# isarandi/metrabs

Hardware: AMD Instinct MI355X
Metric: crops/sec (256px, 72 depth bins) at 1/2/4/8 MI355X; MPJPE vs ref (higher is better)
Workload: dtype f32

## Files before the change

include/metrabs_hip.h:

```cpp
#ifndef METRABS_HIP_H_
#define METRABS_HIP_H_

#include <stddef.h>
#include <stdint.h>

#ifdef __cplusplus
extern "C" {
#endif

#define MTR_VERSION 100

typedef void* mtr_stream_t;

enum mtr_dtype { MTR_F32 = 0, MTR_F16 = 1, MTR_BF16 = 2 };

enum mtr_layout {
  MTR_NCHW = 0,
  MTR_NHWC = 1
};

enum mtr_error {
  MTR_OK = 0,
  MTR_E_NULL = -1,
  MTR_E_SHAPE = -2,
// ... 62 lines not shown
  MTR_HEAD_KERNEL_RT_KS = 3,
  MTR_HEAD_KERNEL_RT_NP = 4,
  MTR_HEAD_KERNEL_16 = 10,
  MTR_HEAD_KERNEL_16_DMA = 11,
  MTR_HEAD_KERNEL_16_DMA_EARLY = 14,
  MTR_HEAD_KERNEL_16_DMA_LOADER = 13,
  MTR_HEAD_KERNEL_16_AREG = 15,
  MTR_HEAD_KERNEL_16_RES = 16,
  MTR_HEAD_KERNEL_16_PP = 17,
  MTR_HEAD_KERNEL_16_DMA_EARLY_TIGHT = 18,
  MTR_HEAD_KERNEL_16_RT = 12
};
typedef struct mtr_head_plan_info {
  int32_t kernel;
  int32_t tiles_per_workgroup;
  int32_t column_blocks;
  int32_t split_column_blocks;
  int64_t workgroups;
  double model_us;
} mtr_head_plan_info;
int mtr_head_plan(int feat_dtype, int layout, int B, int C, int H, int W, int J, int D,
                  const mtr_head_options* options, int have_workspace, mtr_head_plan_info* plan);

size_t mtr_head_workspace_bytes(int feat_dtype, int layout, int B, int C, int H, int W, int J, int D);
int mtr_head_fused_ws(const void* features, int feat_dtype, int layout, int B, int C, int H, int W,
                      const void* packed, int J, int D, const mtr_head_params* p,
                      const mtr_head_options* options, void* workspace, size_t workspace_bytes,
                      float* coords2d, float* coords3d_rel, mtr_stream_t stream);

size_t mtr_reconstruct_workspace_bytes(int B, int J);
int mtr_reconstruct_absolute(const float* coords2d , const float* coords3d_rel ,
                             const float* intrinsics , int B, int J,
                             const mtr_recon_params* p, float* poses3d , void* workspace,
                             size_t workspace_bytes, mtr_stream_t stream);
int mtr_reconstruct_moments(const float* coords2d, const float* coords3d_rel,
                            const float* intrinsics, int B, int J, double* moments ,
                            void* workspace, size_t workspace_bytes, mtr_stream_t stream);
int mtr_reconstruct_solve(const float* coords2d, const float* coords3d_rel, const float* intrinsics,
                          int B, int J, const mtr_recon_params* p, const double* moments ,
                          float* poses3d, mtr_stream_t stream);

#define MTR_WARP_PARAM_FLOATS 36

int mtr_build_pyramid(const uint8_t* images_u8, int N, int Hi, int Wi, float* level0, float* level1,
                      float* level2, mtr_stream_t stream);
int mtr_pyramid_from_level0(const float* level0, int N, int Hi, int Wi, float* level1, float* level2,
                            mtr_stream_t stream);
int mtr_build_pyramid_u8(const uint8_t* images_u8, int N, int Hi, int Wi, float* lut ,
                         float* level1, float* level2, mtr_stream_t stream);
int mtr_warp_crops_u8(const uint8_t* level0_u8, const float* lut, const float* level1,
                      const float* level2, int N, int Hi, int Wi, const float* warp_params,
                      int n_crops, int res, int antialias, int out_dtype, int out_layout, void* out,
                      mtr_stream_t stream);
int mtr_build_pyramid_u8_hwc(const uint8_t* images_u8, int N, int Hi, int Wi, float* lut ,
                             float* level1, float* level2, mtr_stream_t stream);
int mtr_warp_crops_u8_hwc(const uint8_t* level0_u8, const float* lut, const float* level1,
                          const float* level2, int N, int Hi, int Wi, const float* warp_params,
                          int n_crops, int res, int antialias, int out_dtype, int out_layout, void* out,
                          mtr_stream_t stream);
int mtr_crop_geometry(const float* boxes, int box_stride, const float* intrinsics,
                      const float* distortion, const float* camspace_up, const int32_t* image_ids,
                      const float* aug_rotflipmat, const float* aug_scales, const float* aug_gammas,
                      int n_box, int n_aug, int res, int antialias, float* new_intrinsics,
                      float* rot, float* warp_params, mtr_stream_t stream);
int mtr_warp_crops(const float* level0, const float* level1, const float* level2, int N, int Hi,
                   int Wi, const float* warp_params, int n_crops, int res, int antialias,
                   int out_dtype, int out_layout, void* out, mtr_stream_t stream);
size_t mtr_crops_shrink_workspace_bytes(int n_crops, int res, int antialias);
int mtr_crops_shrink_antialiased(const float* crops_big, const float* warp_params, int n_crops, int res,
                                 int antialias, int out_dtype, int out_layout, void* out,
                                 void* workspace, size_t workspace_bytes, mtr_stream_t stream);

int mtr_postprocess_poses(const float* poses_crop, const float* rot, const uint8_t* should_flip,
                          const int32_t* mirror_mapping, const float* joint_transform, int Jt,
                          const int32_t* skeleton, int S, const float* intrinsics,
                          const float* distortion, const float* inv_extrinsics, int A, int n, int J,
                          int average_aug, float* poses3d, float* poses2d, mtr_stream_t stream);

int mtr_linear_combine_points(const float* points, const float* weights, int B, int J_in, int J_out,
                              float* out, mtr_stream_t stream);

typedef struct mtr_detector_geom {
  int32_t target_h, target_w;
  int32_t antialias;
  int32_t pad_top, pad_left;
  int32_t out_h, out_w;
  float x_factor, y_factor;
} mtr_detector_geom;

int mtr_detector_geometry(int H, int W, int input_size , mtr_detector_geom* g);
int mtr_detector_preprocess(const uint8_t* images_u8, int N, int H, int W, const mtr_detector_geom* g,
                            float* out, mtr_stream_t stream);
enum { MTR_DETECTOR_KERNEL_AUTO = 0, MTR_DETECTOR_KERNEL_TILE = 1, MTR_DETECTOR_KERNEL_STREAM = 2 };
int mtr_detector_preprocess_kernel(const uint8_t* images_u8, int N, int H, int W, const mtr_detector_geom* g,
                                   int kernel, float* out, mtr_stream_t stream);
int mtr_detector_scale_boxes(const float* xyxy_conf, int n, const mtr_detector_geom* g,
                             float* boxes_out, mtr_stream_t stream);

typedef struct mtr_filter_params {
  float rel_small, rel_big, abs_diff_mm;
  float stdev_mm;
  float box_fraction;
  float sim_scale_mm, sim_threshold;
  int32_t max_output;
  int32_t var_correction;
  int32_t order_by_score;
} mtr_filter_params;

size_t mtr_filter_poses_workspace_bytes(int P, int J, int max_per_image);
int mtr_filter_poses(const float* poses3d, const float* poses2d, const float* boxes,
                     const int32_t* row_start, const int32_t* sim_offsets, int n_images, int P, int A,
                     int J, const int32_t* edges, const float* mean_bones, int n_bones, int J_model,
                     const mtr_filter_params* params , void* workspace, size_t workspace_bytes,
                     int max_per_image, uint8_t* valid, int32_t* keep_idx, int32_t* keep_count,
                     mtr_stream_t stream);

int mtr_bias_act_nchw(void* y, int dtype, const float* bias , const void* residual, int act,
                      long long B, int C, int HW, mtr_stream_t stream);

int mtr_bias_act_rowmean_nchw(void* y, int dtype, const float* bias , int act, long long B,
                              int C, int HW, float* row_mean , mtr_stream_t stream);

int mtr_depthwise3x3_bias_act(const void* x, int dtype, const float* weight, const float* bias, int act,
                              long long B, int C, int H, int W, int stride, int pad, void* y,
                              float* row_mean, mtr_stream_t stream);
int mtr_depthwise3x3_bias_act_padded(const void* x, int dtype, const float* weight, const float* bias,
                                     int act, long long B, int C, int H, int W, int stride, int pad_top,
                                     int pad_left, int pad_bottom, int pad_right, void* y,
                                     float* row_mean, mtr_stream_t stream);

int mtr_depthwise5x5_bias_act_padded(const void* x, int dtype, const float* weight ,
                                     const float* bias, int act, long long B, int C, int H, int W,
                                     int stride, int pad_top, int pad_left, int pad_bottom, int pad_right,
                                     void* y, float* row_mean , mtr_stream_t stream);

int mtr_se_gate(const float* mean , const float* w1, const float* b1, const float* w2,
                const float* b2, int act, int gate_fn, int B, int C, int S, float* gate ,
                mtr_stream_t stream);

int mtr_conv1x1_bias_act(const void* x, int dtype, const float* weight, const float* bias,
                         const float* gate , const void* residual, int act, long long B,
                         int M, int K, int HW, void* y, mtr_stream_t stream);

int mtr_conv1x1_bias_act16(const void* x, int dtype, const void* weight, const float* bias,
                           const float* gate , const void* residual, int act, long long B,
                           int M, int K, int HW, void* y, mtr_stream_t stream);

int mtr_conv3x3_bias_act16(const void* x, int dtype, const void* weight , const float* bias,
                           const void* residual, int act, long long B, int Cin, int Cout, int H, int W, int stride,
                           void* y, mtr_stream_t stream);

size_t mtr_conv3x3_16_lds_bytes(long long B, int Cin, int Cout, int H, int W, int stride);

#ifdef __cplusplus
}
#endif
#endif
```

metrabs_amd/_lib.py:

```python
import ctypes
import os
from ctypes import POINTER, c_char_p, c_double, c_float, c_int, c_int32, c_size_t, c_uint8, c_void_p

LIB_PATH = os.path.join(os.path.dirname(os.path.abspath(__file__)), 'csrc', 'libmetrabs_hip.so')

MTR_F32, MTR_F16, MTR_BF16 = 0, 1, 2
MTR_NCHW, MTR_NHWC = 0, 1
MTR_WARP_PARAM_FLOATS = 36


class HeadParams(ctypes.Structure):
    _fields_ = [('proc_side', c_int32), ('stride_test', c_int32), ('centered_stride', c_int32),
                ('legacy_centered_stride_bug', c_int32), ('box_size_mm', c_float)]


class HeadOptions(ctypes.Structure):
    _fields_ = [('struct_size', ctypes.c_uint32),
                ('rt_tiles_per_workgroup', c_int32), ('groups_per_workgroup', c_int32),
                ('dma_staging', c_int32), ('rt_column_blocks', c_int32), ('rt_k_groups', c_int32),
                ('rt_loader', c_int32), ('rt_split_column_blocks', c_int32)]


def head_options(rt_tiles=0, groups_per_workgroup=0, dma_staging=-1, rt_column_blocks=0, rt_k_groups=0,
                 rt_loader=0, rt_split=0):
    return HeadOptions(ctypes.sizeof(HeadOptions), int(rt_tiles), int(groups_per_workgroup), int(dma_staging),
                       int(rt_column_blocks), int(rt_k_groups), int(rt_loader), int(rt_split))


class HeadPlanInfo(ctypes.Structure):
    _fields_ = [('kernel', c_int32), ('tiles_per_workgroup', c_int32), ('column_blocks', c_int32),
                ('split_column_blocks', c_int32), ('workgroups', ctypes.c_int64), ('model_us', ctypes.c_double)]


HEAD_KERNEL_NAMES = {1: 'head_rt_kernel', 2: 'head_rt_ld_kernel', 3: 'head_rt_ks_kernel', 4: 'head_rt_np_kernel',
                     10: 'head_fused16_kernel', 11: 'head_fused16dma_kernel', 12: 'head_rt16_kernel',
                     13: 'head_fused16dma_kernel (loader wave)', 14: 'head_fused16dma_kernel (early copies)',
                     15: 'head_fused16areg_kernel (weights in registers)',
                     16: 'head_fused16res_kernel (weights resident, persistent workgroups)',
                     17: 'head_fused16pp_kernel (two alternating halves)',
                     18: 'head_fused16dma_kernel (early copies, tight stage)'}


class ReconParams(ctypes.Structure):
    _fields_ = [('proc_side', c_int32), ('stride_train', c_int32), ('centered_stride', c_int32),
                ('weak_perspective', c_int32), ('mix_enabled', c_int32),
                ('mix_3d_inside_fov', c_float), ('l2_reg', c_float), ('weight_eps', c_float),
                ('fov_border_factor', c_float)]


class DetectorGeom(ctypes.Structure):
    _fields_ = [('target_h', c_int32), ('target_w', c_int32), ('antialias', c_int32),
                ('pad_top', c_int32), ('pad_left', c_int32), ('out_h', c_int32), ('out_w', c_int32),
                ('x_factor', c_float), ('y_factor', c_float)]


class FilterParams(ctypes.Structure):
    _fields_ = [('rel_small', c_float), ('rel_big', c_float), ('abs_diff_mm', c_float),
                ('stdev_mm', c_float), ('box_fraction', c_float), ('sim_scale_mm', c_float),
                ('sim_threshold', c_float), ('max_output', c_int32), ('var_correction', c_int32),
                ('order_by_score', c_int32)]


SIGNATURES = {
    'mtr_version': (c_int, []),
    'mtr_strerror': (c_char_p, [c_int]),
    'mtr_softargmax_decode': (c_int, [c_void_p, c_int, c_int, c_int, c_int, c_int, c_int, c_int,
                                      POINTER(HeadParams), c_void_p, c_void_p, c_void_p]),
    'mtr_softargmax_decode_opts': (c_int, [c_void_p, c_int, c_int, c_int, c_int, c_int, c_int, c_int,
                                           POINTER(HeadParams), c_int, c_void_p, c_void_p, c_void_p]),
    'mtr_head_row_plan': (c_int, [c_int, c_int, POINTER(c_int32), POINTER(c_int32), c_void_p, c_int]),
    'mtr_head_packed_bytes': (c_size_t, [c_int, c_int, c_int, c_int]),
    'mtr_head_pack_weights': (c_int, [c_void_p, c_void_p, c_int, c_int, c_int, c_int, c_void_p,
                                      c_void_p]),
    'mtr_head_fused': (c_int, [c_void_p, c_int, c_int, c_int, c_int, c_int, c_int, c_void_p, c_int,
                               c_int, POINTER(HeadParams), c_void_p, c_void_p, c_void_p]),
    'mtr_head_fused_opts': (c_int, [c_void_p, c_int, c_int, c_int, c_int, c_int, c_int, c_void_p, c_int,
                                    c_int, POINTER(HeadParams), POINTER(HeadOptions), c_void_p, c_void_p,
                                    c_void_p]),
    'mtr_head_plan': (c_int, [c_int, c_int, c_int, c_int, c_int, c_int, c_int, c_int, POINTER(HeadOptions),
                              c_int, POINTER(HeadPlanInfo)]),
    'mtr_head_workspace_bytes': (c_size_t, [c_int, c_int, c_int, c_int, c_int, c_int, c_int, c_int]),
    'mtr_head_fused_ws': (c_int, [c_void_p, c_int, c_int, c_int, c_int, c_int, c_int, c_void_p, c_int,
                                  c_int, POINTER(HeadParams), POINTER(HeadOptions), c_void_p, c_size_t,
                                  c_void_p, c_void_p, c_void_p]),
    'mtr_crops_shrink_workspace_bytes': (c_size_t, [c_int, c_int, c_int]),
    'mtr_crops_shrink_antialiased': (c_int, [c_void_p, c_void_p, c_int, c_int, c_int, c_int, c_int, c_void_p,
                                             c_void_p, c_size_t, c_void_p]),
    'mtr_reconstruct_workspace_bytes': (c_size_t, [c_int, c_int]),
    'mtr_reconstruct_absolute': (c_int, [c_void_p, c_void_p, c_void_p, c_int, c_int,
                                         POINTER(ReconParams), c_void_p, c_void_p, c_size_t,
                                         c_void_p]),
    'mtr_reconstruct_moments': (c_int, [c_void_p, c_void_p, c_void_p, c_int, c_int, c_void_p,
                                        c_void_p, c_size_t, c_void_p]),
    'mtr_reconstruct_solve': (c_int, [c_void_p, c_void_p, c_void_p, c_int, c_int,
                                      POINTER(ReconParams), c_void_p, c_void_p, c_void_p]),
    'mtr_build_pyramid': (c_int, [c_void_p, c_int, c_int, c_int, c_void_p, c_void_p, c_void_p,
                                  c_void_p]),
    'mtr_build_pyramid_u8': (c_int, [c_void_p, c_int, c_int, c_int, c_void_p, c_void_p, c_void_p,
                                     c_void_p]),
    'mtr_warp_crops_u8': (c_int, [c_void_p, c_void_p, c_void_p, c_void_p, c_int, c_int, c_int, c_void_p,
                                  c_int, c_int, c_int, c_int, c_int, c_void_p, c_void_p]),
    'mtr_build_pyramid_u8_hwc': (c_int, [c_void_p, c_int, c_int, c_int, c_void_p, c_void_p, c_void_p,
                                         c_void_p]),
    'mtr_warp_crops_u8_hwc': (c_int, [c_void_p, c_void_p, c_void_p, c_void_p, c_int, c_int, c_int, c_void_p,
                                      c_int, c_int, c_int, c_int, c_int, c_void_p, c_void_p]),
    'mtr_pyramid_from_level0': (c_int, [c_void_p, c_int, c_int, c_int, c_void_p, c_void_p, c_void_p]),
    'mtr_crop_geometry': (c_int, [c_void_p, c_int, c_void_p, c_void_p, c_void_p, c_void_p, c_void_p,
                                  c_void_p, c_void_p, c_int, c_int, c_int, c_int, c_void_p,
                                  c_void_p, c_void_p, c_void_p]),
    'mtr_postprocess_poses': (c_int, [c_void_p, c_void_p, c_void_p, c_void_p, c_void_p, c_int, c_void_p,
                                      c_int, c_void_p, c_void_p, c_void_p, c_int, c_int, c_int, c_int,
                                      c_void_p, c_void_p, c_void_p]),
    'mtr_linear_combine_points': (c_int, [c_void_p, c_void_p, c_int, c_int, c_int, c_void_p, c_void_p]),
    'mtr_warp_crops': (c_int, [c_void_p, c_void_p, c_void_p, c_int, c_int, c_int, c_void_p, c_int,
                               c_int, c_int, c_int, c_int, c_void_p, c_void_p]),
    'mtr_detector_geometry': (c_int, [c_int, c_int, c_int, POINTER(DetectorGeom)]),
    'mtr_detector_preprocess': (c_int, [c_void_p, c_int, c_int, c_int, POINTER(DetectorGeom), c_void_p,
                                        c_void_p]),
    'mtr_detector_preprocess_kernel': (c_int, [c_void_p, c_int, c_int, c_int, POINTER(DetectorGeom), c_int,
                                               c_void_p, c_void_p]),
    'mtr_detector_scale_boxes': (c_int, [c_void_p, c_int, POINTER(DetectorGeom), c_void_p, c_void_p]),
    'mtr_filter_poses_workspace_bytes': (ctypes.c_size_t, [c_int, c_int, c_int]),
    'mtr_filter_poses': (c_int, [c_void_p, c_void_p, c_void_p, c_void_p, c_void_p, c_int, c_int, c_int,
                                 c_int, c_void_p, c_void_p, c_int, c_int, POINTER(FilterParams), c_void_p,
                                 ctypes.c_size_t, c_int, c_void_p, c_void_p, c_void_p, c_void_p]),
    'mtr_depthwise3x3_bias_act': (c_int, [c_void_p, c_int, c_void_p, c_void_p, c_int, ctypes.c_longlong,
                                          c_int, c_int, c_int, c_int, c_int, c_void_p, c_void_p, c_void_p]),
    'mtr_depthwise3x3_bias_act_padded': (c_int, [c_void_p, c_int, c_void_p, c_void_p, c_int, ctypes.c_longlong,
                                                 c_int, c_int, c_int, c_int, c_int, c_int, c_int, c_int,
                                                 c_void_p, c_void_p, c_void_p]),
    'mtr_depthwise5x5_bias_act_padded': (c_int, [c_void_p, c_int, c_void_p, c_void_p, c_int, ctypes.c_longlong,
                                                 c_int, c_int, c_int, c_int, c_int, c_int, c_int, c_int,
                                                 c_void_p, c_void_p, c_void_p]),
    'mtr_bias_act_rowmean_nchw': (c_int, [c_void_p, c_int, c_void_p, c_int, ctypes.c_longlong, c_int, c_int,
                                          c_void_p, c_void_p]),
    'mtr_bias_act_nchw': (c_int, [c_void_p, c_int, c_void_p, c_void_p, c_int, ctypes.c_longlong, c_int,
                                  c_int, c_void_p]),
    'mtr_se_gate': (c_int, [c_void_p, c_void_p, c_void_p, c_void_p, c_void_p, c_int, c_int, c_int, c_int,
                            c_int, c_void_p, c_void_p]),
    'mtr_conv1x1_bias_act': (c_int, [c_void_p, c_int, c_void_p, c_void_p, c_void_p, c_void_p, c_int,
                                     ctypes.c_longlong, c_int, c_int, c_int, c_void_p, c_void_p]),
    'mtr_conv1x1_bias_act16': (c_int, [c_void_p, c_int, c_void_p, c_void_p, c_void_p, c_void_p, c_int,
                                       ctypes.c_longlong, c_int, c_int, c_int, c_void_p, c_void_p]),
    'mtr_conv3x3_bias_act16': (c_int, [c_void_p, c_int, c_void_p, c_void_p, c_void_p, c_int, ctypes.c_longlong,
                                       c_int, c_int, c_int, c_int, c_int, c_void_p, c_void_p]),
    'mtr_conv3x3_16_lds_bytes': (ctypes.c_size_t, [ctypes.c_longlong, c_int, c_int, c_int, c_int, c_int]),
}

_lib = None


def load(path=None):
    global _lib
    if _lib is not None and path is None:
        return _lib
    path = path or LIB_PATH
    import torch
    if not os.path.exists(path):
        raise RuntimeError(
            f'{path} not found: the HIP extension is not built. Run `python -m metrabs_amd.build` '
            f'(needs hipcc). metrabs_amd has no CPU fallback.')
    lib = ctypes.CDLL(path)
    for name, (restype, argtypes) in SIGNATURES.items():
        fn = getattr(lib, name)
        fn.restype = restype
        fn.argtypes = argtypes
    _lib = lib
    return lib


def check(code, what):
    if code != 0:
        msg = load().mtr_strerror(code).decode()
        raise RuntimeError(f'{what} failed: {msg} (code {code})')


def dtype_code(torch_dtype):
    import torch
    try:
        return {torch.float32: MTR_F32, torch.float16: MTR_F16, torch.bfloat16: MTR_BF16}[torch_dtype]
    except KeyError:
        raise TypeError(f'unsupported dtype {torch_dtype}') from None


def current_stream_ptr(device=None):
    import torch
    return c_void_p(torch.cuda.current_stream(device).cuda_stream)


def require_cuda(*tensors):
    for t in tensors:
        if t is not None and not t.is_cuda:
            raise RuntimeError(
                'metrabs_amd kernels run on the GPU only (tensor on %s); there is no CPU fallback'
                % t.device)
```

metrabs_amd/backbones.py:

```python
import collections
import threading

import torch
import torch.nn.functional as F
from torch import nn


class DepthwiseConv2d(nn.Conv2d):

    use_miopen = False
    _backend_lock = threading.Lock()

    def forward(self, x):
        if x.is_cuda and not DepthwiseConv2d.use_miopen and torch.backends.cudnn.enabled:
            cudnn = torch.backends.cudnn
            with DepthwiseConv2d._backend_lock, cudnn.flags(
                    enabled=False, benchmark=cudnn.benchmark, deterministic=cudnn.deterministic,
                    allow_tf32=cudnn.allow_tf32):
                return super().forward(x)
        return super().forward(x)


class ConvBNAct(nn.Sequential):

# ... 207 lines not shown
        return mobilenet_v3_large()
    raise ValueError(f'unknown backbone {name}')


_ACT_NAMES = {nn.SiLU: 'silu', nn.ReLU: 'relu', nn.Hardswish: 'hardswish'}


class ConvBiasAct(nn.Module):

    def __init__(self, conv, bias, act):
        super().__init__()
        self.conv = conv
        self.register_buffer('bias', bias.detach().float().contiguous())
        self.act = act
        self.act_name = None if act is None else _ACT_NAMES[type(act)]
        self.emit_mean = False
        self._mean = None
        self._gate = None
        self.last_path = None

    use_k13 = True
    k13_slower = frozenset({(960, 256, 64), (1536, 256, 64), (256, 1280, 64)})

    def k13_takes(self, x):
        c = self.conv
        if not (ConvBiasAct.use_k13 and not self.emit_mean and x.is_cuda and c.kernel_size == (1, 1)
                and c.stride == (1, 1) and c.padding == (0, 0) and c.dilation == (1, 1) and c.groups == 1
                and c.bias is None and c.padding_mode == 'zeros'):
            return False
        if torch.is_autocast_enabled('cuda') or (torch.is_grad_enabled() and c.weight.requires_grad):
            return False
        if x.dim() != 4 or (c.in_channels, c.out_channels, x.shape[2] * x.shape[3]) in ConvBiasAct.k13_slower:
            return False
        from . import kernels
        return kernels.conv1x1_supported(x, c.weight)

    use_k13h = True
    k13h_slower = frozenset({(192, 48, 4096), (256, 64, 1024), (1536, 256, 64), (256, 64, 9216), (768, 192, 576),
                             (1152, 224, 576), (1344, 224, 576), (1344, 384, 144), (2304, 384, 144),
                             (2304, 640, 144), (640, 3840, 144), (3840, 640, 144), (640, 1280, 144)})

    def k13h_takes(self, x):
        c = self.conv
        if not (ConvBiasAct.use_k13h and not self.emit_mean and x.is_cuda and x.dtype == c.weight.dtype
                and x.dtype in (torch.float16, torch.bfloat16) and c.kernel_size == (1, 1)
                and c.stride == (1, 1) and c.padding == (0, 0) and c.dilation == (1, 1) and c.groups == 1
                and c.bias is None and c.padding_mode == 'zeros'):
            return False
        if torch.is_autocast_enabled('cuda') or (torch.is_grad_enabled() and c.weight.requires_grad):
            return False
        if x.dim() != 4 or (c.in_channels, c.out_channels, x.shape[2] * x.shape[3]) in ConvBiasAct.k13h_slower:
            return False
        from . import kernels
        return kernels.conv1x1_16_supported(x, c.weight)

    def give_gate(self, x, gate):
        self._gate = (x, gate)

    def take_mean_f32(self, x):
        held, self._mean = self._mean, None
        if held is not None and held[0] is x:
            return held[1]
        return None

    def take_mean(self, x):
        m = self.take_mean_f32(x)
        return None if m is None else m.to(x.dtype).view(x.shape[0], x.shape[1], 1, 1)

    def forward(self, x, residual=None):
        held, self._gate = self._gate, None
        gate = held[1] if held is not None and held[0] is x else None
        w16 = self.conv.weight.dtype
        if x.dtype != w16 and w16 in (torch.float16, torch.bfloat16) and not torch.is_autocast_enabled(x.device.type):
            x = x.to(w16)
        if self.k13h_takes(x) and (residual is None or (residual.dtype == x.dtype and residual.is_contiguous()
                                                        and residual.data_ptr() % 16 == 0)):
            from . import kernels
            self.last_path = 'k13h' if gate is None else 'k13h_gate'
            return kernels.conv1x1_bias_act16(x, self.conv.weight, self.bias, self.act_name, gate=gate,
                                              residual=residual)
        if self.k13_takes(x) and (residual is None or (residual.dtype == x.dtype and residual.is_contiguous()
                                                       and residual.data_ptr() % 16 == 0)):
            from . import kernels
            self.last_path = 'k13' if gate is None else 'k13_gate'
            return kernels.conv1x1_bias_act(x, self.conv.weight, self.bias, self.act_name, gate=gate,
                                            residual=residual)
        self.last_path = 'library'
        if gate is not None:
            x = x * gate.to(x.dtype).view(x.shape[0], x.shape[1], 1, 1)
        return _library_conv_bias_act(self, x, residual)


def _library_conv_bias_act(mod, x, residual):
    y = mod.conv(x)
    hw_vec_ok = (y.shape[2] * y.shape[3]) % (16 // y.element_size()) == 0
    if y.is_cuda and y.is_contiguous() and hw_vec_ok and y.data_ptr() % 16 == 0 and (
            residual is None or (residual.dtype == y.dtype and residual.is_contiguous()
                                 and residual.data_ptr() % 16 == 0)):
        from . import kernels
        if getattr(mod, 'emit_mean', False) and residual is None:
            y, mean = kernels.bias_act_rowmean_(y, mod.bias, mod.act_name)
            mod._mean = (y, mean)
            return y
        return kernels.bias_act_(y, mod.bias, mod.act_name, residual)
    y = y + mod.bias.view(1, -1, 1, 1).to(y.dtype)
    y = y if mod.act is None else mod.act(y)
    return y if residual is None else residual + y


class Conv3x3BiasAct(nn.Module):

    use_k14h = True
    k14h_slower = frozenset({(64, 256, 2, 96, 96), (64, 64, 1, 64, 64)})

    def __init__(self, conv, bias, act):
        super().__init__()
        self.conv = conv
        from . import kernels
        self.register_buffer('weight_packed', kernels.pack_conv3x3_weight(conv.weight))
        self.register_buffer('bias', bias.detach().float().contiguous())
        self.act = act
        self.act_name = None if act is None else _ACT_NAMES[type(act)]
        self.stride = conv.stride[0]
        self.last_path = None

    @staticmethod
    def applies_to(conv):
        return (isinstance(conv, nn.Conv2d) and conv.groups == 1 and conv.kernel_size == (3, 3)
                and conv.dilation == (1, 1) and conv.stride in ((1, 1), (2, 2)) and conv.padding == (1, 1)
                and conv.padding_mode == 'zeros' and conv.in_channels % 8 == 0)

    def k14h_takes(self, x):
        c = self.conv
        if not (Conv3x3BiasAct.use_k14h and x.is_cuda and x.dim() == 4 and x.dtype == c.weight.dtype
                and x.dtype in (torch.float16, torch.bfloat16) and c.bias is None):
            return False
        if torch.is_autocast_enabled('cuda') or (torch.is_grad_enabled() and c.weight.requires_grad):
            return False
        if (c.in_channels, c.out_channels, self.stride, x.shape[2], x.shape[3]) in Conv3x3BiasAct.k14h_slower:
            return False
        from . import kernels
        return kernels.conv3x3_16_supported(x, self.weight_packed, self.stride)

    def forward(self, x, residual=None):
        w16 = self.conv.weight.dtype
        if x.dtype != w16 and w16 in (torch.float16, torch.bfloat16) and not torch.is_autocast_enabled(x.device.type):
            x = x.to(w16)
        if self.k14h_takes(x) and (residual is None or (residual.dtype == x.dtype and residual.is_contiguous()
                                                        and residual.data_ptr() % 16 == 0)):
            from . import kernels
            self.last_path = 'k14h'
            return kernels.conv3x3_bias_act16(x, self.weight_packed, self.bias, self.act_name, self.stride,
                                              residual=residual)
        self.last_path = 'library'
        return _library_conv_bias_act(self, x, residual)


class DepthwiseBiasAct(nn.Module):

    kernel_sizes = (3, 5)
    k15_slower = frozenset()

    def __init__(self, conv, bias, act):
        super().__init__()
        self.weight = nn.Parameter(conv.weight.detach().float().contiguous(), requires_grad=False)
        self.register_buffer('bias', bias.detach().float().contiguous())
        self.k = conv.kernel_size[0]
        self.stride, self.pad = conv.stride[0], conv.padding[0]
        self.pads = None
        self.act = act
        self.act_name = None if act is None else _ACT_NAMES[type(act)]
        self.emit_mean = False
        self._mean = None
        self.last_path = None

    @classmethod
    def applies_to(cls, conv):
        k = conv.kernel_size[0] if isinstance(conv, nn.Conv2d) else None
        return (isinstance(conv, nn.Conv2d) and conv.groups == conv.in_channels == conv.out_channels
                and conv.groups > 1 and k in cls.kernel_sizes and conv.kernel_size == (k, k)
                and conv.dilation == (1, 1) and conv.stride in ((1, 1), (2, 2))
                and conv.padding in ((0, 0), (k // 2, k // 2)) and conv.padding_mode == 'zeros')

    take_mean = ConvBiasAct.take_mean
    take_mean_f32 = ConvBiasAct.take_mean_f32

    def forward(self, x):
        pl, pr = (self.pad, self.pad) if self.pads is None else self.pads[:2]
        ow = (x.shape[3] + pl + pr - self.k) // self.stride + 1
        pad = self.pad if self.pads is None else self.pads
        if x.is_cuda and x.is_contiguous() and ow % 4 == 0 and \
                x.dtype in (torch.float32, torch.float16, torch.bfloat16):
            from . import kernels
            if self.k == 3:
                fn, self.last_path = kernels.depthwise3x3_bias_act, 'k11'
            elif (x.shape[1], x.shape[2], x.shape[3], self.stride) not in DepthwiseBiasAct.k15_slower and \
                    kernels.depthwise5x5_supported(x.shape[2], x.shape[3], pad):
                fn, self.last_path = kernels.depthwise5x5_bias_act, 'k15'
            else:
                fn = None
            if fn is not None:
                if self.emit_mean:
                    y, mean = fn(x, self.weight, self.bias, self.act_name, self.stride, pad, want_mean=True)
                    self._mean = (y, mean)
                    return y
                return fn(x, self.weight, self.bias, self.act_name, self.stride, pad)
        self.last_path = 'library'
        if self.pads is not None:
            x = F.pad(x, self.pads)
        y = F.conv2d(x, self.weight.to(x.dtype), self.bias.to(x.dtype), self.stride,
                     self.pad if self.pads is None else 0, groups=self.weight.shape[0])
        return y if self.act is None else self.act(y)


def _block_plus_skip(block, x):
    last = block[-1]
    tail = last[0] if isinstance(last, ConvBNAct) else None
    if isinstance(tail, (ConvBiasAct, Conv3x3BiasAct)):
        y = x
        for m in list(block)[:-1]:
            y = m(y)
        for m in list(last)[1:]:
            assert isinstance(m, nn.Identity)
        return tail(y, residual=x)
    return x + block(x)


def fold_batchnorm(backbone, fused_epilogue=False, dtype=None):
    import copy
    from torch.nn.utils.fusion import fuse_conv_bn_eval
    if backbone.training:
        raise ValueError('fold_batchnorm needs the running statistics of an eval-mode network')
    if dtype not in (None, torch.float16, torch.bfloat16):
        raise ValueError(f'fold_batchnorm: dtype must be None, torch.float16 or torch.bfloat16, got {dtype}')
    if dtype is not None and not fused_epilogue:
        raise ValueError('fold_batchnorm: a 16-bit copy (dtype=) needs fused_epilogue=True')
    folded = copy.deepcopy(backbone)
    for m in folded.modules():
        if isinstance(m, ConvBNAct) and isinstance(m[1], nn.BatchNorm2d):
            conv = fuse_conv_bn_eval(m[0], m[1])
            act = m[2] if len(m) > 2 else None
            if fused_epilogue and (act is None or type(act) in _ACT_NAMES):
                bias, conv.bias = conv.bias, None
                m[0] = (DepthwiseBiasAct if DepthwiseBiasAct.applies_to(conv) else ConvBiasAct)(
                    conv, bias, act)
                if act is not None:
                    m[2] = nn.Identity()
            else:
                m[0] = conv
            m[1] = nn.Identity()
    if any(isinstance(m, nn.BatchNorm2d) for m in folded.modules()):
        raise ValueError('a BatchNorm2d outside a ConvBNAct block cannot be folded here')
    if fused_epilogue:
        for seq in folded.modules():
            if not isinstance(seq, nn.Sequential) or isinstance(seq, ConvBNAct):
                continue
            names = list(seq._modules)
            for n_pad, n_conv in zip(names, names[1:]):
                pad, blk = seq._modules[n_pad], seq._modules[n_conv]
                if isinstance(pad, nn.ZeroPad2d) and isinstance(blk, ConvBNAct) and \
                        isinstance(blk[0], DepthwiseBiasAct) and blk[0].pad == 0:
                    l, r, t, b = (int(p) for p in pad.padding)
                    lo, hi = blk[0].k // 2, blk[0].k // 2 + 1
                    if 0 <= l <= lo and 0 <= t <= lo and 0 <= r <= hi and 0 <= b <= hi:
                        blk[0].pads = (l, r, t, b)
                        seq._modules[n_pad] = nn.Identity()
    if fused_epilogue:
        for seq in folded.modules():
            if not isinstance(seq, nn.Sequential) or isinstance(seq, ConvBNAct):
                continue
            kids = list(seq)
            for prev, nxt in zip(kids, kids[1:]):
                if isinstance(nxt, SqueezeExcite) and isinstance(prev, ConvBNAct) and \
                        isinstance(prev[0], (ConvBiasAct, DepthwiseBiasAct)) and \
                        all(isinstance(m, nn.Identity) for m in list(prev)[1:]):
                    prev[0].emit_mean = True
                    nxt.mean_from = (prev[0],)
        for seq in folded.modules():
            if not isinstance(seq, nn.Sequential) or isinstance(seq, ConvBNAct):
                continue
            kids = list(seq)
            for prev, nxt in zip(kids, kids[1:]):
                if isinstance(prev, SqueezeExcite) and isinstance(nxt, ConvBNAct) and \
                        isinstance(nxt[0], ConvBiasAct):
                    prev.gate_to = (nxt[0],)
    if dtype is not None:
        for m in folded.modules():
            if isinstance(m, ConvBiasAct):
                m.conv.to(dtype)
        for m in folded.modules():
            if isinstance(m, ConvBNAct) and isinstance(m[0], ConvBiasAct) and not m[0].emit_mean \
                    and Conv3x3BiasAct.applies_to(m[0].conv):
                m[0] = Conv3x3BiasAct(m[0].conv, m[0].bias, m[0].act)
        folded.inference_dtype = dtype
    return folded


def calibrate_batchnorm(backbone, res, dev, batches=2, batch_size=16, seed=7, samples=None):
    bns = [m for m in backbone.modules() if isinstance(m, torch.nn.BatchNorm2d)]
    for m in bns:
        m.momentum = None
        m.reset_running_stats()
    backbone.train()
    g = torch.Generator(device=dev).manual_seed(seed)
    with torch.no_grad():
        for _ in range(batches):
            backbone(torch.rand(batch_size, 3, res, res, device=dev, generator=g))
        if samples is not None:
            for chunk in samples.float().split(batch_size):
                if len(chunk) > 1:
                    backbone(chunk)
    backbone.eval()
    return backbone
```

metrabs_amd/kernels.py:

```python
import ctypes

import torch

from metrabs_amd import _lib
from metrabs_amd._lib import check, current_stream_ptr, dtype_code, require_cuda


def _ptr(t):
    return ctypes.c_void_p(t.data_ptr()) if t is not None else ctypes.c_void_p(0)


def softargmax_decode(logits, n_points, cfg, out=None, nhwc_staging=0):
    require_cuda(logits)
    lib = _lib.load()
    nhwc = _is_channels_last(logits)
    if not nhwc:
        logits = logits.contiguous()
    B, n_out, H, W = logits.shape
    J = int(n_points)
    D = n_out // J - 1
    if n_out != J * (1 + D) or D != cfg.depth:
        raise ValueError(f'logits have {n_out} channels, expected J*(1+depth) = {J * (1 + cfg.depth)}')
    if out is None:
        c2d = torch.empty(B, J, 2, device=logits.device, dtype=torch.float32)
# ... 488 lines not shown


def depthwise5x5_bias_act(x, weight, bias, act, stride, pad, want_mean=False):
    require_cuda(x, weight, bias)
    if not x.is_contiguous():
        raise ValueError('depthwise5x5_bias_act needs an NCHW-contiguous tensor')
    if weight.numel() != x.shape[1] * 25:
        raise ValueError(f'depthwise5x5_bias_act needs a [C, 5, 5] weight, got {tuple(weight.shape)}')
    B, C, H, W = x.shape
    pl, pr, pt, pb = (pad,) * 4 if isinstance(pad, int) else tuple(int(p) for p in pad)
    OH, OW = (H + pt + pb - 5) // stride + 1, (W + pl + pr - 5) // stride + 1
    y = torch.empty(B, C, max(OH, 0), max(OW, 0), device=x.device, dtype=x.dtype)
    mean = torch.empty(B, C, device=x.device, dtype=torch.float32) if want_mean else None
    check(_lib.load().mtr_depthwise5x5_bias_act_padded(
        _ptr(x), dtype_code(x.dtype), _ptr(weight.contiguous().float()), _ptr(bias.contiguous().float()),
        ACT_CODES[act], B, C, H, W, int(stride), pt, pl, pb, pr, _ptr(y), None if mean is None else _ptr(mean),
        current_stream_ptr(x.device)), 'mtr_depthwise5x5_bias_act_padded')
    return (y, mean) if want_mean else y



SE_GATE_CODES = {'sigmoid': 0, 'hardsigmoid': 1}


def se_gate(mean, w1, b1, w2, b2, act, gate_fn, out=None):
    require_cuda(mean, w1, b1, w2, b2)
    B, C = mean.shape[0], mean.shape[1]
    S = w1.shape[0]
    w1, w2 = w1.reshape(S, -1), w2.reshape(C, -1)
    if mean.dtype != torch.float32 or mean.numel() != B * C or w1.shape[1] != C or w2.shape[1] != S:
        raise ValueError('se_gate: mean [B, C] f32, w1 [S, C], w2 [C, S]')
    tensors = [t.contiguous().float() for t in (mean, w1, b1, w2, b2)]
    if out is None:
        out = torch.empty(B, C, device=mean.device, dtype=torch.float32)
    check(_lib.load().mtr_se_gate(*(_ptr(t) for t in tensors), ACT_CODES[act], SE_GATE_CODES[gate_fn], B, C, S,
                                  _ptr(out), current_stream_ptr(mean.device)), 'mtr_se_gate')
    return out



def conv1x1_supported(x, weight):
    if x.dim() != 4 or x.dtype != torch.float32 or weight.dtype != torch.float32 or not x.is_contiguous():
        return False
    K, HW = x.shape[1], x.shape[2] * x.shape[3]
    return (weight.numel() == weight.shape[0] * K and HW % 4 == 0 and K % 4 == 0
            and x.data_ptr() % 16 == 0 and weight.data_ptr() % 16 == 0
            and x.shape[0] * HW < 2 ** 31 and K * HW < 2 ** 31 and weight.shape[0] * HW < 2 ** 31)


def conv1x1_bias_act(x, w, bias, act, gate=None, residual=None, out=None):
    require_cuda(x, w, bias, gate, residual)
    B, K, H, W = x.shape
    M = w.shape[0]
    w = w.reshape(M, -1)
    if w.shape[1] != K:
        raise ValueError(f'conv1x1_bias_act: weight has {w.shape[1]} input channels, x has {K}')
    if gate is not None and (gate.dtype != torch.float32 or gate.numel() != B * K):
        raise ValueError('conv1x1_bias_act: gate must be [B, Cin] f32')
    if residual is not None and (residual.shape != (B, M, H, W) or residual.dtype != x.dtype
                                 or not residual.is_contiguous()):
        raise ValueError('conv1x1_bias_act: residual must be [B, Cout, H, W] like the output, contiguous')
    if out is None:
        out = torch.empty(B, M, H, W, device=x.device, dtype=x.dtype)
    elif out.shape != (B, M, H, W) or out.dtype != x.dtype or not out.is_contiguous():
        raise ValueError('conv1x1_bias_act: out must be [B, Cout, H, W] like the output, contiguous')
    check(_lib.load().mtr_conv1x1_bias_act(
        _ptr(x), dtype_code(x.dtype), _ptr(w.contiguous()), _ptr(bias.contiguous().float()),
        None if gate is None else _ptr(gate.contiguous()), None if residual is None else _ptr(residual),
        ACT_CODES[act], B, M, K, H * W, _ptr(out), current_stream_ptr(x.device)), 'mtr_conv1x1_bias_act')
    return out



def conv1x1_16_supported(x, weight):
    if x.dim() != 4 or x.dtype not in (torch.float16, torch.bfloat16) or weight.dtype != x.dtype \
            or not x.is_contiguous() or not weight.is_contiguous():
        return False
    K, HW = x.shape[1], x.shape[2] * x.shape[3]
    return (weight.numel() == weight.shape[0] * K and HW % 8 == 0 and K % 8 == 0
            and x.data_ptr() % 16 == 0 and weight.data_ptr() % 16 == 0
            and x.shape[0] * HW < 2 ** 31 and K * HW < 2 ** 31 and weight.shape[0] * HW < 2 ** 31)


def conv1x1_bias_act16(x, w, bias, act, gate=None, residual=None, out=None):
    require_cuda(x, w, bias, gate, residual)
    B, K, H, W = x.shape
    M = w.shape[0]
    w = w.reshape(M, -1)
    if w.shape[1] != K:
        raise ValueError(f'conv1x1_bias_act16: weight has {w.shape[1]} input channels, x has {K}')
    if w.dtype != x.dtype:
        raise ValueError(f'conv1x1_bias_act16: weight is {w.dtype}, x is {x.dtype}')
    if gate is not None and (gate.dtype != torch.float32 or gate.numel() != B * K):
        raise ValueError('conv1x1_bias_act16: gate must be [B, Cin] f32')
    if residual is not None and (residual.shape != (B, M, H, W) or residual.dtype != x.dtype
                                 or not residual.is_contiguous()):
        raise ValueError('conv1x1_bias_act16: residual must be [B, Cout, H, W] like the output, contiguous')
    if out is None:
        out = torch.empty(B, M, H, W, device=x.device, dtype=x.dtype)
    elif out.shape != (B, M, H, W) or out.dtype != x.dtype or not out.is_contiguous():
        raise ValueError('conv1x1_bias_act16: out must be [B, Cout, H, W] like the output, contiguous')
    check(_lib.load().mtr_conv1x1_bias_act16(
        _ptr(x), dtype_code(x.dtype), _ptr(w.contiguous()), _ptr(bias.contiguous().float()),
        None if gate is None else _ptr(gate.contiguous()), None if residual is None else _ptr(residual),
        ACT_CODES[act], B, M, K, H * W, _ptr(out), current_stream_ptr(x.device)), 'mtr_conv1x1_bias_act16')
    return out



def pack_conv3x3_weight(weight):
    if weight.dim() != 4 or tuple(weight.shape[2:]) != (3, 3):
        raise ValueError(f'pack_conv3x3_weight: expected [Cout, Cin, 3, 3], got {tuple(weight.shape)}')
    return weight.detach().permute(0, 2, 3, 1).contiguous()


def conv3x3_16_supported(x, weight, stride):
    if x.dim() != 4 or weight.dim() != 4 or x.dtype not in (torch.float16, torch.bfloat16) \
            or weight.dtype != x.dtype or not x.is_contiguous() or x.data_ptr() % 16 or weight.data_ptr() % 16:
        return False
    B, K, H, W = x.shape
    if weight.numel() != weight.shape[0] * K * 9 or B >= 2 ** 16:
        return False
    return _lib.load().mtr_conv3x3_16_lds_bytes(B, K, weight.shape[0], H, W, int(stride)) > 0


def conv3x3_bias_act16(x, w_packed, bias, act, stride, residual=None, out=None):
    require_cuda(x, w_packed, bias, residual)
    if x.dim() != 4 or not x.is_contiguous():
        raise ValueError('conv3x3_bias_act16: x must be [B, Cin, H, W], NCHW-contiguous')
    B, K, H, W = x.shape
    M = w_packed.shape[0]
    if w_packed.dim() != 4 or tuple(w_packed.shape[1:]) != (3, 3, K) or not w_packed.is_contiguous():
        raise ValueError(f'conv3x3_bias_act16: the weight must be packed [Cout, 3, 3, {K}] and contiguous, '
                         f'got {tuple(w_packed.shape)}')
    if w_packed.dtype != x.dtype:
        raise ValueError(f'conv3x3_bias_act16: weight is {w_packed.dtype}, x is {x.dtype}')
    if stride not in (1, 2):
        raise ValueError(f'conv3x3_bias_act16: stride must be 1 or 2, got {stride}')
    if bias.numel() != M:
        raise ValueError(f'conv3x3_bias_act16: bias has {bias.numel()} elements, expected {M}')
    Ho, Wo = (H - 1) // stride + 1, (W - 1) // stride + 1
    if residual is not None and (residual.shape != (B, M, Ho, Wo) or residual.dtype != x.dtype
                                 or not residual.is_contiguous()):
        raise ValueError('conv3x3_bias_act16: residual must be [B, Cout, Ho, Wo] like the output, contiguous')
    if out is None:
        out = torch.empty(B, M, Ho, Wo, device=x.device, dtype=x.dtype)
    elif out.shape != (B, M, Ho, Wo) or out.dtype != x.dtype or not out.is_contiguous():
        raise ValueError('conv3x3_bias_act16: out must be [B, Cout, Ho, Wo] like the output, contiguous')
    check(_lib.load().mtr_conv3x3_bias_act16(
        _ptr(x), dtype_code(x.dtype), _ptr(w_packed), _ptr(bias.contiguous().float()),
        None if residual is None else _ptr(residual), ACT_CODES[act], B, K, M, H, W, int(stride), _ptr(out),
        current_stream_ptr(x.device)), 'mtr_conv3x3_bias_act16')
    return out
```

Measured before the change: 8268.

## Add fused f32 MFMA implicit-GEMM 3x3 conv with bias, activation and residual

Adds a new HIP kernel that computes 3x3 convolutions in f32 as an implicit GEMM on MFMA 32x32x2 f32 instructions. It stages a haloed, channel-interleaved input tile in LDS and prefetches weights in registers, then fuses bias, activation and residual add into the epilogue. The f32 fused-epilogue fold path now swaps eligible ConvBiasAct 3x3 layers to this kernel instead of the library conv. This removes separate library conv and epilogue launches, at the cost of a large LDS footprint that may limit occupancy, and the build must compile the new source file.

```diff
diff --git a/include/metrabs_hip.h b/include/metrabs_hip.h
--- a/include/metrabs_hip.h
+++ b/include/metrabs_hip.h
@@ -238,6 +238,12 @@
 
 size_t mtr_conv3x3_16_lds_bytes(long long B, int Cin, int Cout, int H, int W, int stride);
 
+int mtr_conv3x3_bias_act(const float* x, const float* weight , const float* bias,
+                         const float* residual, int act, long long B, int Cin, int Cout, int H, int W, int stride,
+                         float* y, mtr_stream_t stream);
+
+size_t mtr_conv3x3_lds_bytes(long long B, int Cin, int Cout, int H, int W, int stride);
+
 #ifdef __cplusplus
 }
 #endif
diff --git a/metrabs_amd/_lib.py b/metrabs_amd/_lib.py
--- a/metrabs_amd/_lib.py
+++ b/metrabs_amd/_lib.py
@@ -145,6 +145,9 @@
     'mtr_conv3x3_bias_act16': (c_int, [c_void_p, c_int, c_void_p, c_void_p, c_void_p, c_int, ctypes.c_longlong,
                                        c_int, c_int, c_int, c_int, c_int, c_void_p, c_void_p]),
     'mtr_conv3x3_16_lds_bytes': (ctypes.c_size_t, [ctypes.c_longlong, c_int, c_int, c_int, c_int, c_int]),
+    'mtr_conv3x3_bias_act': (c_int, [c_void_p, c_void_p, c_void_p, c_void_p, c_int, ctypes.c_longlong,
+                                     c_int, c_int, c_int, c_int, c_int, c_void_p, c_void_p]),
+    'mtr_conv3x3_lds_bytes': (ctypes.c_size_t, [ctypes.c_longlong, c_int, c_int, c_int, c_int, c_int]),
 }
 
 _lib = None
diff --git a/metrabs_amd/backbones.py b/metrabs_amd/backbones.py
--- a/metrabs_amd/backbones.py
+++ b/metrabs_amd/backbones.py
@@ -383,6 +383,52 @@
             self.last_path = 'k14h'
             return kernels.conv3x3_bias_act16(x, self.weight_packed, self.bias, self.act_name, self.stride,
                                               residual=residual)
+        self.last_path = 'library'
+        return _library_conv_bias_act(self, x, residual)
+
+
+class Conv3x3BiasActF32(nn.Module):
+
+    use_k14 = True
+    k14_slower = frozenset()
+
+    def __init__(self, conv, bias, act):
+        super().__init__()
+        self.conv = conv
+        from . import kernels
+        self.register_buffer('weight_packed', kernels.pack_conv3x3_weight(conv.weight).float())
+        self.register_buffer('bias', bias.detach().float().contiguous())
+        self.act = act
+        self.act_name = None if act is None else _ACT_NAMES[type(act)]
+        self.stride = conv.stride[0]
+        self.last_path = None
+
+    @staticmethod
+    def applies_to(conv):
+        return (isinstance(conv, nn.Conv2d) and conv.groups == 1 and conv.kernel_size == (3, 3)
+                and conv.dilation == (1, 1) and conv.stride in ((1, 1), (2, 2)) and conv.padding == (1, 1)
+                and conv.padding_mode == 'zeros' and conv.in_channels % 4 == 0
+                and conv.weight.dtype == torch.float32)
+
+    def k14_takes(self, x):
+        c = self.conv
+        if not (Conv3x3BiasActF32.use_k14 and x.is_cuda and x.dim() == 4 and x.dtype == torch.float32
+                and c.weight.dtype == torch.float32 and c.bias is None):
+            return False
+        if torch.is_autocast_enabled('cuda') or (torch.is_grad_enabled() and c.weight.requires_grad):
+            return False
+        if (c.in_channels, c.out_channels, self.stride, x.shape[2], x.shape[3]) in Conv3x3BiasActF32.k14_slower:
+            return False
+        from . import kernels
+        return kernels.conv3x3_supported(x, self.weight_packed, self.stride)
+
+    def forward(self, x, residual=None):
+        if self.k14_takes(x) and (residual is None or (residual.dtype == x.dtype and residual.is_contiguous()
+                                                       and residual.data_ptr() % 16 == 0)):
+            from . import kernels
+            self.last_path = 'k14'
+            return kernels.conv3x3_bias_act(x, self.weight_packed, self.bias, self.act_name, self.stride,
+                                            residual=residual)
         self.last_path = 'library'
         return _library_conv_bias_act(self, x, residual)
 
@@ -447,7 +493,7 @@
 def _block_plus_skip(block, x):
     last = block[-1]
     tail = last[0] if isinstance(last, ConvBNAct) else None
-    if isinstance(tail, (ConvBiasAct, Conv3x3BiasAct)):
+    if isinstance(tail, (ConvBiasAct, Conv3x3BiasAct, Conv3x3BiasActF32)):
         y = x
         for m in list(block)[:-1]:
             y = m(y)
@@ -524,6 +570,11 @@
                     and Conv3x3BiasAct.applies_to(m[0].conv):
                 m[0] = Conv3x3BiasAct(m[0].conv, m[0].bias, m[0].act)
         folded.inference_dtype = dtype
+    elif fused_epilogue:
+        for m in folded.modules():
+            if isinstance(m, ConvBNAct) and isinstance(m[0], ConvBiasAct) and not m[0].emit_mean \
+                    and Conv3x3BiasActF32.applies_to(m[0].conv):
+                m[0] = Conv3x3BiasActF32(m[0].conv, m[0].bias, m[0].act)
     return folded
 
 
diff --git a/metrabs_amd/csrc/conv3x3.hip b/metrabs_amd/csrc/conv3x3.hip
--- /dev/null
+++ b/metrabs_amd/csrc/conv3x3.hip
@@ -0,0 +1,293 @@
+#include "common.h"
+
+namespace mtr {
+
+typedef float c3f_f32x16 __attribute__((ext_vector_type(16)));
+
+template <int V> struct Conv3fActTag { static constexpr int value = V; };
+
+struct Conv3fGeo {
+  int Cin, M, H, W, Ho, Wo, stride;
+  int lw;
+  int tiles_x;
+  int HH, LW;
+  int LDC;
+};
+
+constexpr int kConv3fLoadUnroll = 4;
+constexpr int kConv3fPrefetch = 2;
+
+template <int WM, int WN, int FM, int FN>
+__global__ __launch_bounds__(64 * WM * WN) void conv3x3_f32_kernel(
+    const float* __restrict__ x, const float* __restrict__ w, const float* __restrict__ bias,
+    const float* __restrict__ residual, float* __restrict__ y, Conv3fGeo g, int act) {
+  constexpr int NT = 64 * WM * WN;
+  constexpr int BM = 32 * FM * WM, BN = 32 * FN * WN;
+  constexpr int U = kConv3fLoadUnroll;
+  extern __shared__ __attribute__((aligned(16))) float xs[];
+
+  const int tid = threadIdx.x, lane = tid & 63, wave = tid >> 6;
+  const int wm = wave % WM, wn = wave / WM;
+  const int r = lane & 31, h = lane >> 5;
+  const int Cin = g.Cin, M = g.M, H = g.H, W = g.W, s = g.stride, LW = g.LW, LDC = g.LDC;
+  const int TW = 1 << g.lw;
+  const int tile_y = blockIdx.x / g.tiles_x, tile_x = blockIdx.x - tile_y * g.tiles_x;
+  const int oy0 = tile_y * (BN >> g.lw), ox0 = tile_x * TW, m0 = blockIdx.y * BM;
+  const long long b = blockIdx.z, plane = (long long)H * W;
+
+  {
+    const float* xb = x + b * Cin * plane;
+    const int iy0 = oy0 * s - 1, ix0 = ox0 * s - 4;
+    const int GW = LW >> 2, n_units = 4 * GW * g.HH * ((Cin + 15) >> 4);
+    for (int u0 = 0; u0 < n_units; u0 += U * NT) {
+      float4 v[U][4];
+      int dst[U];
+#pragma unroll
+      for (int k = 0; k < U; ++k) {
+        const int u = u0 + k * NT + tid;
+        dst[k] = -1;
+#pragma unroll
+        for (int i = 0; i < 4; ++i) v[k][i] = make_float4(0.0f, 0.0f, 0.0f, 0.0f);
+        if (u < n_units) {
+          const int rest = u >> 2, gx = rest % GW, rest2 = rest / GW, ly = rest2 % g.HH;
+          const int c4 = (rest2 / g.HH) * 4 + (u & 3);
+          if (4 * c4 < Cin) {
+            dst[k] = (ly * LW + 4 * gx) * LDC + 4 * c4;
+            const int iy = iy0 + ly, ix = ix0 + 4 * gx;
+            if (iy >= 0 && iy < H && ix >= 0 && ix < W) {
+              const float* p = xb + (long long)(4 * c4) * plane + (long long)iy * W + ix;
+#pragma unroll
+              for (int i = 0; i < 4; ++i) v[k][i] = *reinterpret_cast<const float4*>(p + i * plane);
+            }
+          }
+        }
+      }
+#pragma unroll
+      for (int k = 0; k < U; ++k) {
+        if (dst[k] < 0) continue;
+        float* d = xs + dst[k];
+        *reinterpret_cast<float4*>(d) = make_float4(v[k][0].x, v[k][1].x, v[k][2].x, v[k][3].x);
+        *reinterpret_cast<float4*>(d + LDC) = make_float4(v[k][0].y, v[k][1].y, v[k][2].y, v[k][3].y);
+        *reinterpret_cast<float4*>(d + 2 * LDC) = make_float4(v[k][0].z, v[k][1].z, v[k][2].z, v[k][3].z);
+        *reinterpret_cast<float4*>(d + 3 * LDC) = make_float4(v[k][0].w, v[k][1].w, v[k][2].w, v[k][3].w);
+      }
+    }
+  }
+
+  const int G4 = Cin >> 2, NG = 9 * G4, n_steps = (NG + 1) >> 1;
+  const long long K9 = 9LL * Cin;
+  int abase[FN];
+#pragma unroll
+  for (int j = 0; j < FN; ++j) {
+    const int p = (wn * FN + j) * 32 + r, oyl = p >> g.lw, oxl = p & (TW - 1);
+    abase[j] = ((oyl * s) * LW + oxl * s + 3) * LDC;
+  }
+  const float* wrow[FM];
+#pragma unroll
+  for (int i = 0; i < FM; ++i) {
+    const int m = m0 + (wm * FM + i) * 32 + r;
+    wrow[i] = w + (m < M ? m : 0) * K9;
+  }
+  auto load_w = [&](float4 (&wr)[FM], int grp) {
+    const int gq = grp < NG ? grp : NG - 1;
+#pragma unroll
+    for (int i = 0; i < FM; ++i) wr[i] = *reinterpret_cast<const float4*>(wrow[i] + 4 * gq);
+  };
+
+  c3f_f32x16 acc[FM][FN];
+#pragma unroll
+  for (int i = 0; i < FM; ++i)
+#pragma unroll
+    for (int j = 0; j < FN; ++j)
+#pragma unroll
+      for (int e = 0; e < 16; ++e) acc[i][j][e] = 0.0f;
+
+  int grp = h, tap = h / G4, c4 = h - tap * G4;
+  constexpr int D = kConv3fPrefetch;
+  float4 wq[D][FM];
+#pragma unroll
+  for (int d = 0; d < D; ++d) load_w(wq[d], grp + 2 * d);
+  __syncthreads();
+  for (int step = 0; step < n_steps; step += D) {
+#pragma unroll
+    for (int d = 0; d < D; ++d) {
+      if (step + d >= n_steps) break;
+      const bool valid = grp < NG;
+      const int ky = tap / 3, kx = tap - 3 * ky;
+      const int toff = valid ? (ky * LW + kx) * LDC + 4 * c4 : 0;
+      float4 a[FN];
+#pragma unroll
+      for (int j = 0; j < FN; ++j) {
+        a[j] = *reinterpret_cast<const float4*>(xs + abase[j] + toff);
+        if (!valid) a[j] = make_float4(0.0f, 0.0f, 0.0f, 0.0f);
+      }
+      float4 wv[FM];
+#pragma unroll
+      for (int i = 0; i < FM; ++i) wv[i] = valid ? wq[d][i] : make_float4(0.0f, 0.0f, 0.0f, 0.0f);
+#pragma unroll
+      for (int i = 0; i < FM; ++i)
+#pragma unroll
+        for (int j = 0; j < FN; ++j) acc[i][j] = __builtin_amdgcn_mfma_f32_32x32x2f32(a[j].x, wv[i].x, acc[i][j], 0, 0, 0);
+#pragma unroll
+      for (int i = 0; i < FM; ++i)
+#pragma unroll
+        for (int j = 0; j < FN; ++j) acc[i][j] = __builtin_amdgcn_mfma_f32_32x32x2f32(a[j].y, wv[i].y, acc[i][j], 0, 0, 0);
+#pragma unroll
+      for (int i = 0; i < FM; ++i)
+#pragma unroll
+        for (int j = 0; j < FN; ++j) acc[i][j] = __builtin_amdgcn_mfma_f32_32x32x2f32(a[j].z, wv[i].z, acc[i][j], 0, 0, 0);
+#pragma unroll
+      for (int i = 0; i < FM; ++i)
+#pragma unroll
+        for (int j = 0; j < FN; ++j) acc[i][j] = __builtin_amdgcn_mfma_f32_32x32x2f32(a[j].w, wv[i].w, acc[i][j], 0, 0, 0);
+      load_w(wq[d], grp + 2 * D);
+      grp += 2;
+      c4 += 2;
+      if (c4 >= G4) { c4 -= G4; ++tap; }
+      if (c4 >= G4) { c4 -= G4; ++tap; }
+    }
+  }
+
+  auto epilogue = [&](auto tag) {
+    constexpr int ACT = decltype(tag)::value;
+#pragma unroll
+    for (int i = 0; i < FM; ++i) {
+      const int m = m0 + (wm * FM + i) * 32 + r;
+      if (m >= M) continue;
+      const float bm = bias[m];
+      const long long chan = (b * M + m) * (long long)g.Ho * g.Wo;
+#pragma unroll
+      for (int j = 0; j < FN; ++j) {
+#pragma unroll
+        for (int q = 0; q < 4; ++q) {
+          const int p = (wn * FN + j) * 32 + 8 * q + 4 * h;
+          const int oy = oy0 + (p >> g.lw), ox = ox0 + (p & (TW - 1));
+          if (oy >= g.Ho || ox >= g.Wo) continue;
+          const long long at = chan + (long long)oy * g.Wo + ox;
+          float4 o;
+          o.x = activate<ACT>(acc[i][j][4 * q + 0] + bm);
+          o.y = activate<ACT>(acc[i][j][4 * q + 1] + bm);
+          o.z = activate<ACT>(acc[i][j][4 * q + 2] + bm);
+          o.w = activate<ACT>(acc[i][j][4 * q + 3] + bm);
+          if (residual) {
+            const float4 t = *reinterpret_cast<const float4*>(residual + at);
+            o.x += t.x, o.y += t.y, o.z += t.z, o.w += t.w;
+          }
+          *reinterpret_cast<float4*>(y + at) = o;
+        }
+      }
+    }
+  };
+  switch (act) {
+    case kActRelu: epilogue(Conv3fActTag<kActRelu>()); break;
+    case kActSilu: epilogue(Conv3fActTag<kActSilu>()); break;
+    case kActHardswish: epilogue(Conv3fActTag<kActHardswish>()); break;
+    default: epilogue(Conv3fActTag<kActNone>()); break;
+  }
+}
+
+constexpr size_t kConv3fMaxLds = 160 * 1024;
+constexpr size_t kConv3fWantLds = 80 * 1024;
+
+static void conv3x3_f32_geometry(Conv3fGeo& g, int BN) {
+  long long best = -1;
+  for (int lw = 6; lw >= 3; --lw) {
+    const int TW = 1 << lw, TH = BN >> lw;
+    if (TH < 1) continue;
+    const long long padded = (long long)((g.Wo + TW - 1) / TW) * TW * (((g.Ho + TH - 1) / TH) * TH);
+    if (best < 0 || padded < best) {
+      best = padded;
+      g.lw = lw;
+    }
+  }
+  const int TW = 1 << g.lw, TH = BN >> g.lw;
+  g.tiles_x = (g.Wo + TW - 1) / TW;
+  g.HH = (TH - 1) * g.stride + 3;
+  g.LW = 4 * (((TW - 1) * g.stride + 6 + 3) / 4);
+  g.LDC = g.Cin + ((g.Cin & 4) ? 0 : 4);
+}
+
+template <int WM, int WN, int FM, int FN>
+static size_t conv3x3_f32_cfg_lds(Conv3fGeo g) {
+  conv3x3_f32_geometry(g, 32 * FN * WN);
+  return (size_t)g.HH * g.LW * g.LDC * sizeof(float);
+}
+
+template <int WM, int WN, int FM, int FN>
+static int launch_conv3x3_f32_cfg(const float* x, const float* w, const float* bias, const float* residual, float* y,
+                                  int act, long long B, Conv3fGeo g, hipStream_t stream) {
+  constexpr int BM = 32 * FM * WM, BN = 32 * FN * WN;
+  conv3x3_f32_geometry(g, BN);
+  const size_t lds = (size_t)g.HH * g.LW * g.LDC * sizeof(float);
+  if (lds > kConv3fMaxLds) return MTR_E_SHAPE;
+  const int TH = BN >> g.lw;
+  const long long gx = (long long)g.tiles_x * ((g.Ho + TH - 1) / TH), gy = (g.M + BM - 1) / BM;
+  if (gx > 0x7fffffffLL || gy > 65535 || B > 65535) return MTR_E_SHAPE;
+  if (!y) return (int)lds;
+  auto kern = conv3x3_f32_kernel<WM, WN, FM, FN>;
+  if (lds > 64 * 1024) {
+    const int e = allow_dynamic_lds((const void*)kern, kConv3fMaxLds);
+    if (e != MTR_OK) return e;
+  }
+  const dim3 grid((unsigned)gx, (unsigned)gy, (unsigned)B), block(64 * WM * WN);
+  MTR_CLEAR_STALE();
+  hipLaunchKernelGGL(kern, grid, block, lds, stream, x, w, bias, residual, y, g, act);
+  MTR_CHECK_LAUNCH();
+  return MTR_OK;
+}
+
+template <int WM, int WN, int FM, int FN, int FN_NARROW>
+static int launch_conv3x3_f32_pair(const float* x, const float* w, const float* bias, const float* residual, float* y,
+                                   int act, long long B, const Conv3fGeo& g, hipStream_t s) {
+  const size_t wide = conv3x3_f32_cfg_lds<WM, WN, FM, FN>(g), narrow = conv3x3_f32_cfg_lds<WM, WN, FM, FN_NARROW>(g);
+  if (wide > kConv3fWantLds && (narrow <= kConv3fWantLds || wide > kConv3fMaxLds))
+    return launch_conv3x3_f32_cfg<WM, WN, FM, FN_NARROW>(x, w, bias, residual, y, act, B, g, s);
+  return launch_conv3x3_f32_cfg<WM, WN, FM, FN>(x, w, bias, residual, y, act, B, g, s);
+}
+
+static int launch_conv3x3_f32(const float* x, const float* w, const float* bias, const float* residual, float* y,
+                              int act, long long B, const Conv3fGeo& g, hipStream_t s) {
+  const int M = g.M;
+  if (M <= 32) return launch_conv3x3_f32_pair<1, 4, 1, 2, 1>(x, w, bias, residual, y, act, B, g, s);
+  if (M <= 96) return launch_conv3x3_f32_pair<1, 4, 3, 2, 1>(x, w, bias, residual, y, act, B, g, s);
+  if ((M > 128 && M <= 192) || M % 192 == 0)
+    return launch_conv3x3_f32_pair<2, 2, 3, 2, 1>(x, w, bias, residual, y, act, B, g, s);
+  return launch_conv3x3_f32_pair<2, 2, 2, 2, 1>(x, w, bias, residual, y, act, B, g, s);
+}
+
+static int conv3x3_f32_shape(Conv3fGeo& g, long long B, int Cin, int Cout, int H, int W, int stride) {
+  if (B < 0 || Cin <= 0 || Cout <= 0 || H <= 0 || W <= 0) return MTR_E_SHAPE;
+  if (stride != 1 && stride != 2) return MTR_E_SHAPE;
+  const int Ho = (H - 1) / stride + 1, Wo = (W - 1) / stride + 1;
+  if (Cin % 4 || W % 4 || Wo % 4) return MTR_E_SHAPE;
+  if ((long long)Cin * H * W > 0x7fffffffLL || (long long)Cout * Ho * Wo > 0x7fffffffLL || Cin > 4096)
+    return MTR_E_SHAPE;
+  g = Conv3fGeo{};
+  g.Cin = Cin, g.M = Cout, g.H = H, g.W = W, g.Ho = Ho, g.Wo = Wo, g.stride = stride;
+  return MTR_OK;
+}
+
+}
+
+extern "C" size_t mtr_conv3x3_lds_bytes(long long B, int Cin, int Cout, int H, int W, int stride) {
+  mtr::Conv3fGeo g;
+  if (mtr::conv3x3_f32_shape(g, B, Cin, Cout, H, W, stride) != MTR_OK) return 0;
+  const int n = mtr::launch_conv3x3_f32(nullptr, nullptr, nullptr, nullptr, nullptr, 0, B, g, nullptr);
+  return n > 0 ? (size_t)n : 0;
+}
+
+extern "C" int mtr_conv3x3_bias_act(const float* x, const float* weight, const float* bias, const float* residual,
+                                    int act, long long B, int Cin, int Cout, int H, int W, int stride, float* y,
+                                    mtr_stream_t stream) {
+  if (!x || !weight || !bias || !y) return MTR_E_NULL;
+  mtr::Conv3fGeo g;
+  const int e = mtr::conv3x3_f32_shape(g, B, Cin, Cout, H, W, stride);
+  if (e != MTR_OK) return e;
+  if (act < mtr::kActNone || act > mtr::kActHardswish) return MTR_E_PARAM;
+  if (((uintptr_t)x % 16) || ((uintptr_t)weight % 16) || ((uintptr_t)y % 16) || ((uintptr_t)residual % 16) ||
+      ((uintptr_t)bias % 4))
+    return MTR_E_ALIGN;
+  if (x == y || residual == y) return MTR_E_PARAM;
+  if (B == 0) return mtr_conv3x3_lds_bytes(1, Cin, Cout, H, W, stride) ? MTR_OK : MTR_E_SHAPE;
+  return mtr::launch_conv3x3_f32(x, weight, bias, residual, y, act, B, g, (hipStream_t)stream);
+}
diff --git a/metrabs_amd/kernels.py b/metrabs_amd/kernels.py
--- a/metrabs_amd/kernels.py
+++ b/metrabs_amd/kernels.py
@@ -664,3 +664,46 @@
         None if residual is None else _ptr(residual), ACT_CODES[act], B, K, M, H, W, int(stride), _ptr(out),
         current_stream_ptr(x.device)), 'mtr_conv3x3_bias_act16')
     return out
+
+
+
+def conv3x3_supported(x, weight, stride):
+    if x.dim() != 4 or weight.dim() != 4 or x.dtype != torch.float32 or weight.dtype != torch.float32 \
+            or not x.is_contiguous() or x.data_ptr() % 16 or weight.data_ptr() % 16:
+        return False
+    B, K, H, W = x.shape
+    if weight.numel() != weight.shape[0] * K * 9 or B >= 2 ** 16:
+        return False
+    return _lib.load().mtr_conv3x3_lds_bytes(B, K, weight.shape[0], H, W, int(stride)) > 0
+
+
+def conv3x3_bias_act(x, w_packed, bias, act, stride, residual=None, out=None):
+    require_cuda(x, w_packed, bias, residual)
+    if x.dim() != 4 or not x.is_contiguous() or x.dtype != torch.float32:
+        raise ValueError('conv3x3_bias_act: x must be f32 [B, Cin, H, W], NCHW-contiguous')
+    B, K, H, W = x.shape
+    M = w_packed.shape[0]
+    if w_packed.dim() != 4 or tuple(w_packed.shape[1:]) != (3, 3, K) or not w_packed.is_contiguous():
+        raise ValueError(f'conv3x3_bias_act: the weight must be packed [Cout, 3, 3, {K}] and contiguous, '
+                         f'got {tuple(w_packed.shape)}')
+    if w_packed.dtype != x.dtype:
+        raise ValueError(f'conv3x3_bias_act: weight is {w_packed.dtype}, x is {x.dtype}')
+    if stride not in (1, 2):
+        raise ValueError(f'conv3x3_bias_act: stride must be 1 or 2, got {stride}')
+    if bias.numel() != M:
+        raise ValueError(f'conv3x3_bias_act: bias has {bias.numel()} elements, expected {M}')
+    Ho, Wo = (H - 1) // stride + 1, (W - 1) // stride + 1
+    if residual is not None and (residual.shape != (B, M, Ho, Wo) or residual.dtype != x.dtype
+                                 or not residual.is_contiguous()):
+        raise ValueError('conv3x3_bias_act: residual must be [B, Cout, Ho, Wo] like the output, contiguous')
+    if out is None:
+        out = torch.empty(B, M, Ho, Wo, device=x.device, dtype=x.dtype)
+    elif out.shape != (B, M, Ho, Wo) or out.dtype != x.dtype or not out.is_contiguous():
+        raise ValueError('conv3x3_bias_act: out must be [B, Cout, Ho, Wo] like the output, contiguous')
+    if bias.dtype != torch.float32 or not bias.is_contiguous():
+        bias = bias.contiguous().float()
+    check(_lib.load().mtr_conv3x3_bias_act(
+        _ptr(x), _ptr(w_packed), _ptr(bias), None if residual is None else _ptr(residual),
+        ACT_CODES[act], B, K, M, H, W, int(stride), _ptr(out), current_stream_ptr(x.device)),
+        'mtr_conv3x3_bias_act')
+    return out
```

Result: faster. 8653 (median of 6 runs) (+4.7%).
